# m4tx/idencomp

Measured on NVIDIA B200. Metric: fastq_compress_decompress_GBps, higher is better.
Workload: dtype u32

## Files before the change

idencomp_b200/csrc/idn_gpu.cu:

```cuda
#include "../../include/idn_gpu.h"

#include <algorithm>
#include <cstdarg>
#include <cstdio>
#include <chrono>
#include <cstring>
#include <string>
#include <vector>

#include "idn_fastq.cuh"
#include "idn_native.cuh"

using namespace idn;

namespace {

struct DevBuf {
    void* p = nullptr;
    size_t cap = 0;
    cudaError_t ensure(size_t n) {
        if (n <= cap) return cudaSuccess;
        if (p) cudaFree(p);
        p = nullptr;
        cap = 0;
// ... 36 lines not shown
        cudaFree(d_hvals);
        cudaFree(d_enc);
        cudaFree(d_dec);
        cudaFree(d_adirect);
        cudaFree(d_aenc);
        cudaFree(d_qwin);
        d_qwin = d_aenc = nullptr;
        d_map = d_hkeys = d_hvals = d_enc = d_dec = d_adirect = nullptr;
        used = false;
    }
};

constexpr uint32_t kMaxSlots = 1024;
constexpr uint64_t kDenseSpecLimit = 1ull << 22;
constexpr uint64_t kDirectSpecLimit = 1ull << 19;

}

struct idn_gpu_pipe;

struct idn_gpu_ctx {
    int device = 0;
    idn_gpu_pipe* pipe = nullptr;
    uint32_t pipe_blocks = 32;
    bool pipe_blocks_set = false;
    uint32_t* pipe_err_out = nullptr;
    cudaStream_t stream = nullptr;
    cudaEvent_t ev = nullptr;
    std::string err;
    uint64_t launches = 0;
    bool profiling = false;
    std::vector<cudaEvent_t> prof_pool;
    size_t prof_used = 0;
    struct ProfMark {
        const char* name;
        cudaEvent_t ev;
    };
    std::vector<ProfMark> prof_marks;
    struct HostPhase {
        const char* name;
        uint64_t n;
        double ms;
    };
    std::vector<HostPhase> host_phases;
    std::vector<ModelSlot> slots;
    ModelDev* d_models = nullptr;
    ModelDev d_models_host0{};
    int sm_count = 148;
    int32_t walk_mode = 0;
    uint32_t* d_crc_tab = nullptr;
    uint32_t* d_xpow = nullptr;
    uint32_t* d_crc_back = nullptr;
    bool enc_crc = true;
    DevBuf w_scratch, w_paylen, w_sizes, w_chosen, w_tiles, w_sliceoff, w_readblock, w_small, w_crcpart, w_crclen;
    DevBuf w_walkdone, w_blockadj;
    DevBuf w_lanefirst, w_laneoff, w_laneblock, w_blkinfo, w_nhdr, w_lanesym;
    uint32_t lane_syms = 2048;
    DevBuf f_text, f_tilecnt, f_tilebase, f_linestart, f_linefn, f_linestate, f_tilefn, f_tilestate, f_recscan, f_title, f_namelo,
        f_namelen, f_readlen, f_readoff, f_nameoff, f_names, f_acids, f_quals, f_err, f_fmtoff, f_fmttext;
    idn_fastq_info f_info{};
    uint64_t f_consumed = 0;
    DevBuf f_blockfirst, f_nxt;
    uint32_t f_blocks = 0;
    uint64_t f_reads_used = 0;
    DevBuf w_index;
    DevBuf w_blk;
    DevBuf s_acids, s_quals, s_readoff, s_blockfirst, s_prefix, s_names, s_nameoff, s_out, s_blockoff, s_crc, s_stats,
        s_sizes, s_blocks, s_blocklen, s_aout, s_qout, s_offout, s_status, s_idx;
    DevBuf w_bucket, w_list;
    bool bucket_pairs = true;
    uint64_t resident_bytes = 0;
    uint32_t resident_blocks = 0;
};

namespace {

int32_t fail(idn_gpu_ctx* c, int32_t code, const char* fmt, ...) {
    if (c) {
        char buf[512];
        va_list ap;
        va_start(ap, fmt);
        vsnprintf(buf, sizeof buf, fmt, ap);
        va_end(ap);
        c->err = buf;
    }
    return code;
}

#define CU(call)                                                                                       \
    do {                                                                                               \
        cudaError_t e__ = (call);                                                                      \
        if (e__ != cudaSuccess) {                                                                      \
            (void)cudaGetLastError();                                                                  \
            return fail(ctx, IDN_E_CUDA, "%s failed: %s (%s:%d)", #call, cudaGetErrorString(e__), __FILE__, \
                        __LINE__);                                                                     \
        }                                                                                              \
    } while (0)

#define LAUNCHED(name)                                                                             \
    do {                                                                                           \
        ctx->launches++;                                                                           \
        if (ctx->profiling) prof_mark(ctx, name, st);                                              \
        cudaError_t e__ = cudaGetLastError();                                                      \
        if (e__ != cudaSuccess)                                                                    \
            return fail(ctx, IDN_E_CUDA, "kernel launch failed: %s (%s:%d)", cudaGetErrorString(e__), \
                        __FILE__, __LINE__);                                                       \
// ... 88 lines not shown

using SP0 = StaticSpecs<1, 8, 0, 0, 1, 0, 0, 2, 6, 0>;
using SP1 = StaticSpecs<1, 8, 0, 0, 1, 0, 2, 1, 6, 0>;
using SP2 = StaticSpecs<0, 8, 0, 0, 0, 1, 0, 4, 0, 16>;
using SP3 = StaticSpecs<1, 4, 3, 2, 8, 1, 0, 4, 3, 16>;
using SP4 = StaticSpecs<0, 4, 1, 2, 0, 1, 0, 4, 3, 16>;
using SP5 = StaticSpecs<0, 8, 0, 0, 0, 1, 2, 4, 2, 8>;
using SP6 = StaticSpecs<0, 8, 0, 0, 0, 1, 0, 3, 0, 32>;
using SP7 = StaticSpecs<0, 8, 0, 0, 0, 1, 0, 4, 3, 16>;
constexpr int kNumStaticPairs = 8;
static const int32_t kStaticPairs[kNumStaticPairs][10] = {
    {1, 8, 0, 0, 1, 0, 0, 2, 6, 0}, {1, 8, 0, 0, 1, 0, 2, 1, 6, 0}, {0, 8, 0, 0, 0, 1, 0, 4, 0, 16}, {1, 4, 3, 2, 8, 1, 0, 4, 3, 16},
    {0, 4, 1, 2, 0, 1, 0, 4, 3, 16}, {0, 8, 0, 0, 0, 1, 2, 4, 2, 8}, {0, 8, 0, 0, 0, 1, 0, 3, 0, 32}, {0, 8, 0, 0, 0, 1, 0, 4, 3, 16}};

static int static_pair_index(const idn_gpu_ctx* ctx, int32_t acid_slot, int32_t q_slot) {
    if (!ctx->slots[acid_slot].dev.map || !ctx->slots[q_slot].dev.map || !ctx->slots[acid_slot].dev.adirect || !ctx->slots[q_slot].dev.qwin) return -1;
#ifndef IDN_NO_AENC
    if (!ctx->slots[acid_slot].dev.aenc) return -1;
#endif
    for (int i = 0; i < kNumStaticPairs; i++) {
        bool same = true;
        for (int k = 0; k < 5; k++)
            same = same && ctx->slots[acid_slot].spec_tuple[k] == kStaticPairs[i][k] && ctx->slots[q_slot].spec_tuple[k] == kStaticPairs[i][5 + k];
        if (same) return i;
    }
    return -1;
}

extern "C" int32_t idn_gpu_kernel_variant(const idn_gpu_ctx* ctx, idn_model_t acid_model, idn_model_t q_model) {
    if (!ctx) return -1;
    for (idn_model_t h : {acid_model, q_model})
        if (h < 0 || (size_t)h >= ctx->slots.size() || !ctx->slots[h].used) return -1;
    if (ctx->slots[acid_model].dev.type != IDN_MODEL_ACID || ctx->slots[q_model].dev.type != IDN_MODEL_QSCORE) return -1;
    return static_pair_index(ctx, acid_model, q_model);
}
extern "C" int32_t idn_gpu_kernel_variant_count(void) { return kNumStaticPairs; }

static unsigned debug_smem() {
    static const unsigned v = [] { const char* e = getenv("IDN_DEBUG_SMEM"); return e ? (unsigned)atoi(e) : 0u; }();
    return v;
}
#define IDN_LAUNCH_UNIFORM(idx, KERNEL, grid, st, ...)                                         \
    switch (idx) {                                                                             \
        case 0: KERNEL<true, SP0><<<grid, 128, debug_smem(), st>>>(__VA_ARGS__); break;                   \
        case 1: KERNEL<true, SP1><<<grid, 128, debug_smem(), st>>>(__VA_ARGS__); break;                   \
        case 2: KERNEL<true, SP2><<<grid, 128, debug_smem(), st>>>(__VA_ARGS__); break;                   \
        case 3: KERNEL<true, SP3><<<grid, 128, debug_smem(), st>>>(__VA_ARGS__); break;                   \
        case 4: KERNEL<true, SP4><<<grid, 128, debug_smem(), st>>>(__VA_ARGS__); break;                   \
        case 5: KERNEL<true, SP5><<<grid, 128, debug_smem(), st>>>(__VA_ARGS__); break;                   \
        case 6: KERNEL<true, SP6><<<grid, 128, debug_smem(), st>>>(__VA_ARGS__); break;                   \
        case 7: KERNEL<true, SP7><<<grid, 128, debug_smem(), st>>>(__VA_ARGS__); break;                   \
        default: KERNEL<true, DynSpecs><<<grid, 128, debug_smem(), st>>>(__VA_ARGS__); break;             \
    }

#define IDN_LAUNCH_LIST(idx, KERNEL, grid, st, ...)                                            \
    switch (idx) {                                                                             \
        case 0: KERNEL<SP0><<<grid, 128, debug_smem(), st>>>(__VA_ARGS__); break;                         \
        case 1: KERNEL<SP1><<<grid, 128, debug_smem(), st>>>(__VA_ARGS__); break;                         \
        case 2: KERNEL<SP2><<<grid, 128, debug_smem(), st>>>(__VA_ARGS__); break;                         \
        case 3: KERNEL<SP3><<<grid, 128, debug_smem(), st>>>(__VA_ARGS__); break;                         \
        case 4: KERNEL<SP4><<<grid, 128, debug_smem(), st>>>(__VA_ARGS__); break;                         \
        case 5: KERNEL<SP5><<<grid, 128, debug_smem(), st>>>(__VA_ARGS__); break;                         \
        case 6: KERNEL<SP6><<<grid, 128, debug_smem(), st>>>(__VA_ARGS__); break;                         \
        case 7: KERNEL<SP7><<<grid, 128, debug_smem(), st>>>(__VA_ARGS__); break;                         \
        default: KERNEL<DynSpecs><<<grid, 128, debug_smem(), st>>>(__VA_ARGS__); break;                   \
    }

extern "C" int32_t idn_gpu_abi_version(void) { return IDN_GPU_ABI_VERSION; }

extern "C" int32_t idn_gpu_device_count(void) {
    int n = 0;
    if (cudaGetDeviceCount(&n) != cudaSuccess) {
        (void)cudaGetLastError();
        return 0;
    }
    return n;
}

static void make_crc_tables(uint32_t* tab, uint32_t* xpow) {
    for (uint32_t i = 0; i < 256; i++) {
        uint32_t c = i;
        for (int k = 0; k < 8; k++) c = (c >> 1) ^ ((c & 1) ? 0xEDB88320u : 0);
        tab[i] = c;
    }
    auto mul = [](uint32_t a, uint32_t b) {
        uint32_t p = 0;
        for (int i = 0; i < 32; i++) {
            if (b & 0x80000000u) p ^= a;
            a = (a >> 1) ^ ((a & 1) ? 0xEDB88320u : 0);
            b <<= 1;
        }
        return p;
    };
    xpow[0] = 0x00800000u;
    for (int k = 1; k < 64; k++) xpow[k] = mul(xpow[k - 1], xpow[k - 1]);
}

static void make_crc_back_tables(const uint32_t* tab, const uint32_t* xpow, uint32_t* back ) {
    uint32_t rtop[256];
    for (uint32_t i = 0; i < 256; i++) rtop[tab[i] >> 24] = i;
    uint32_t* tinv = back;
    uint32_t* u = back + 256;
    for (uint32_t t = 0; t < 256; t++) tinv[t] = (tab[rtop[t]] << 8) | rtop[t];
    auto linv = [&](uint32_t v) { return (v << 8) ^ tinv[v >> 24]; };
    for (uint32_t b = 0; b < 256; b++) u[b] = linv(tab[b]);
    auto mul = [](uint32_t a, uint32_t b) {
// ... 1 lines not shown
        for (int i = 0; i < 32; i++) {
            if (b & 0x80000000u) p ^= a;
            a = (a >> 1) ^ ((a & 1) ? 0xEDB88320u : 0);
            b <<= 1;
        }
        return p;
    };
    uint32_t* xlen = back + 512;
    uint32_t x = 0x80000000u;
    for (uint32_t n = 0; n < kCrcLenTab; n++) {
        xlen[2 * n] = x;
        xlen[2 * n + 1] = mul(x, x);
        x = mul(x, xpow[0]);
    }
}

extern "C" int32_t idn_gpu_create(int32_t device, idn_gpu_ctx** out) {
    if (!out) return IDN_E_INVALID_ARG;
    *out = nullptr;
    int n = idn_gpu_device_count();
    if (n <= 0 || device < 0 || device >= n) return IDN_E_CUDA;
    idn_gpu_ctx* ctx = new idn_gpu_ctx();
    ctx->device = device;
    if (const char* pb = getenv("IDN_PIPE_BLOCKS")) {
        ctx->pipe_blocks = std::max(1, atoi(pb));
        ctx->pipe_blocks_set = true;
    }
    if (getenv("IDN_NO_BUCKETS")) ctx->bucket_pairs = false;
    if (const char* w = getenv("IDN_WALK")) ctx->walk_mode = strcmp(w, "serial") == 0 ? 1 : (strcmp(w, "fast") == 0 ? 2 : 0);
    auto bail = [&](const char* what) {
        fprintf(stderr, "idn_gpu_create: %s failed: %s\n", what, cudaGetErrorString(cudaGetLastError()));
        delete ctx;
        return (int32_t)IDN_E_CUDA;
    };
    if (cudaSetDevice(device) != cudaSuccess) return bail("cudaSetDevice");
    if (cudaDeviceGetAttribute(&ctx->sm_count, cudaDevAttrMultiProcessorCount, device) != cudaSuccess) return bail("cudaDeviceGetAttribute");
    if (cudaStreamCreateWithFlags(&ctx->stream, cudaStreamNonBlocking) != cudaSuccess) return bail("cudaStreamCreate");
    if (cudaEventCreateWithFlags(&ctx->ev, cudaEventDisableTiming | cudaEventBlockingSync) != cudaSuccess) return bail("cudaEventCreate");
    if (cudaMalloc(&ctx->d_models, sizeof(ModelDev) * kMaxSlots) != cudaSuccess) return bail("cudaMalloc");
    if (cudaMemset(ctx->d_models, 0, sizeof(ModelDev) * kMaxSlots) != cudaSuccess) return bail("cudaMemset");
    uint32_t tab[256], xpow[64];
    make_crc_tables(tab, xpow);
    if (cudaMalloc(&ctx->d_crc_tab, sizeof tab) != cudaSuccess) return bail("cudaMalloc");
    if (cudaMalloc(&ctx->d_xpow, sizeof xpow) != cudaSuccess) return bail("cudaMalloc");
    if (cudaMemcpy(ctx->d_crc_tab, tab, sizeof tab, cudaMemcpyHostToDevice) != cudaSuccess) return bail("cudaMemcpy");
    if (cudaMemcpy(ctx->d_xpow, xpow, sizeof xpow, cudaMemcpyHostToDevice) != cudaSuccess) return bail("cudaMemcpy");
    {
        std::vector<uint32_t> back(512 + 2 * kCrcLenTab);
        make_crc_back_tables(tab, xpow, back.data());
        if (cudaMalloc(&ctx->d_crc_back, back.size() * 4) != cudaSuccess) return bail("cudaMalloc");
        if (cudaMemcpy(ctx->d_crc_back, back.data(), back.size() * 4, cudaMemcpyHostToDevice) != cudaSuccess) return bail("cudaMemcpy");
    }
    if (getenv("IDN_NO_ENC_CRC")) ctx->enc_crc = false;
    *out = ctx;
    return IDN_OK;
}

static void pipe_destroy(idn_gpu_pipe* p);

extern "C" void idn_gpu_destroy(idn_gpu_ctx* ctx) {
    if (!ctx) return;
    cudaSetDevice(ctx->device);
    cudaDeviceSynchronize();
    for (auto& s : ctx->slots)
        if (s.used) s.free_all();
    DevBuf* bufs[] = {&ctx->w_scratch, &ctx->w_paylen,  &ctx->w_sizes,   &ctx->w_chosen,     &ctx->w_tiles,  &ctx->w_sliceoff,
                      &ctx->w_readblock, &ctx->w_small, &ctx->w_crcpart, &ctx->w_crclen,     &ctx->w_index,  &ctx->w_blk,
                      &ctx->w_lanefirst, &ctx->w_laneoff, &ctx->w_laneblock, &ctx->w_blkinfo, &ctx->w_nhdr, &ctx->w_lanesym, &ctx->w_walkdone, &ctx->w_blockadj,
                      &ctx->f_text, &ctx->f_tilecnt, &ctx->f_tilebase, &ctx->f_linestart, &ctx->f_linefn, &ctx->f_linestate, &ctx->f_tilefn,
                      &ctx->f_tilestate, &ctx->f_recscan, &ctx->f_title, &ctx->f_namelo, &ctx->f_namelen, &ctx->f_readlen, &ctx->f_readoff,
                      &ctx->f_nameoff, &ctx->f_names, &ctx->f_acids, &ctx->f_quals, &ctx->f_err, &ctx->f_fmtoff, &ctx->f_fmttext,
                      &ctx->f_blockfirst, &ctx->f_nxt, &ctx->w_bucket, &ctx->w_list,
                      &ctx->s_acids,   &ctx->s_quals,   &ctx->s_readoff, &ctx->s_blockfirst, &ctx->s_prefix, &ctx->s_names,
                      &ctx->s_nameoff, &ctx->s_out,     &ctx->s_blockoff, &ctx->s_crc,       &ctx->s_stats,  &ctx->s_sizes,
                      &ctx->s_blocks,  &ctx->s_blocklen, &ctx->s_aout,    &ctx->s_qout,    &ctx->s_offout,     &ctx->s_status, &ctx->s_idx};
    for (DevBuf* b : bufs) b->release();
    pipe_destroy(ctx->pipe);
    cudaFree(ctx->d_models);
    cudaFree(ctx->d_crc_tab);
    cudaFree(ctx->d_xpow);
    cudaFree(ctx->d_crc_back);
    if (ctx->ev) cudaEventDestroy(ctx->ev);
    if (ctx->stream) cudaStreamDestroy(ctx->stream);
    delete ctx;
}

extern "C" int32_t idn_gpu_host_alloc(uint64_t bytes, void** p) {
    if (!p) return IDN_E_INVALID_ARG;
    *p = nullptr;
    if (cudaHostAlloc(p, bytes ? bytes : 1, cudaHostAllocPortable) != cudaSuccess) {
        (void)cudaGetLastError();
        *p = nullptr;
        return IDN_E_CUDA;
    }
    return IDN_OK;
}
extern "C" void idn_gpu_host_free(void* p) {
    if (p) cudaFreeHost(p);
}

extern "C" int32_t idn_gpu_set_walk(idn_gpu_ctx* ctx, int32_t mode) {
    if (!ctx) return IDN_E_INVALID_ARG;
    if (mode < 0 || mode > 2) return fail(ctx, IDN_E_INVALID_ARG, "walk mode %d", mode);
    ctx->walk_mode = mode;
    return IDN_OK;
}
// ... 328 lines not shown
                                   uint32_t* block_crc, idn_compress_stats* stats_dev, cudaStream_t st);


extern "C" int32_t idn_gpu_compress_blocks_dev(idn_gpu_ctx* ctx, const idn_batch* batch, int32_t mode,
                                               const idn_model_t* models, uint32_t n_models, int32_t fast,
                                               const uint32_t* prefix_len, uint8_t* out, uint64_t out_cap,
                                               uint64_t* block_off, uint32_t* block_crc, idn_compress_stats* stats_dev,
                                               void* stream) {
    if (!ctx) return IDN_E_INVALID_ARG;
    int32_t rc = check_batch(ctx, batch);
    if (rc) return rc;
    rc = check_models(ctx, models, n_models);
    if (rc) return rc;
    if (mode != IDN_MODE_COMPAT && mode != IDN_MODE_NATIVE) return fail(ctx, IDN_E_UNSUPPORTED, "unknown mode %d", mode);
    if (!batch->block_first_read || !block_off || (!out && out_cap)) return fail(ctx, IDN_E_INVALID_ARG, "NULL argument");
    if (batch->n_blocks == 0) return fail(ctx, IDN_E_INVALID_ARG, "batch has no blocks");
    CU(cudaSetDevice(ctx->device));
    cudaStream_t st = as_stream(stream);
    PROF_BEGIN();
    const uint64_t R = batch->n_reads, S = batch->n_symbols;
    const uint32_t B = batch->n_blocks;
    const bool fuse_crc = ctx->enc_crc && batch->names == nullptr && R > 0;

    SmallParams sp;
    memset(&sp, 0, sizeof sp);
    uint32_t n_score = 0;
    for (uint32_t i = 0; i < n_models; i++) {
        uint32_t t = ctx->slots[models[i]].dev.type;
        if (sp.n_cand[t] >= (uint32_t)kMaxCand) return fail(ctx, IDN_E_UNSUPPORTED, "more than %d models of one type", kMaxCand);
        uint32_t k = sp.n_cand[t]++;
        sp.cand_model[t * kMaxCand + k] = models[i];
        sp.cand_index[t * kMaxCand + k] = (uint8_t)i;
    }
    if (R > 0 && (sp.n_cand[0] == 0 || sp.n_cand[1] == 0))
        return fail(ctx, IDN_E_INVALID_STATE, "need at least one acid model and one quality score model");
    if (fast && n_models != 2) return fail(ctx, IDN_E_INVALID_STATE, "fast mode needs exactly 2 models (compressor_block.rs:96)");
    for (uint32_t t = 0; t < 2; t++) {
        sp.has_sizes[t] = !fast && sp.n_cand[t] > 1;
        if (sp.has_sizes[t])
            for (uint32_t k = 0; k < sp.n_cand[t]; k++) {
                sp.cand_cols[t * kMaxCand + k] = n_score;
                sp.score_ids[n_score++] = sp.cand_model[t * kMaxCand + k];
            }
    }
    if (mode == IDN_MODE_NATIVE) return compress_native_dev(ctx, batch, sp, fast, prefix_len, out, out_cap, block_off, block_crc, stats_dev, st);
    rc = upload_small(ctx, sp, st);
    if (rc) return rc;
    SmallParams* dsp = ctx->w_small.as<SmallParams>();

    CU(ctx->w_scratch.ensure(4 * S + kSlotExtra * R + 16));
    CU(ctx->w_paylen.ensure((R + 1) * 4));
    CU(ctx->w_sliceoff.ensure((R + 2) * 8));
    CU(ctx->w_readblock.ensure((R + 1) * 4));
    const uint32_t n_tiles = (uint32_t)((R + kScanTile - 1) / kScanTile);
    CU(ctx->w_tiles.ensure(((size_t)n_tiles + 2) * 8));
    uint8_t* chosen = nullptr;
    uint8_t* switched = nullptr;
    if (!fast) {
        CU(ctx->w_chosen.ensure(4 * R + 16));
        chosen = ctx->w_chosen.as<uint8_t>();
        switched = chosen + 2 * R;
    }

    if (R > 0) {
        if (n_score) {
            CU(ctx->w_sizes.ensure(R * n_score * 4));
            rc = launch_score(ctx, sp.score_ids, n_score, batch, n_score, ctx->w_sizes.as<uint32_t>(), &dsp->err, st);
            if (rc) return rc;
        }
        if (!fast && n_score == 0) {
            CU(cudaMemsetAsync(chosen, 0, 4 * R, st));
            switch_single_kernel<<<(B + 127) / 128, 128, 0, st>>>(batch->block_first_read, B, switched, R);
            LAUNCHED("switch_single");
        } else if (!fast) {
            switch_kernel<<<2 * B, 32, 0, st>>>(ctx->w_sizes.as<uint32_t>(), n_score, dsp->cand_cols, dsp->n_cand,
                                                dsp->has_sizes, batch->block_first_read, B, chosen, switched, R);
            LAUNCHED("switch");
        }
        EncodeArgs ea;
        ea.models = ctx->d_models;
        ea.acids = batch->acids;
        ea.quals = batch->quals;
        ea.n_symbols = S;
        ea.read_off = batch->read_off;
        ea.n_reads = R;
        ea.fixed_acid = sp.cand_model[0];
        ea.fixed_q = sp.cand_model[kMaxCand];
        ea.chosen = chosen;
        ea.cand_model = dsp->cand_model;
        ea.scratch = ctx->w_scratch.as<uint8_t>();
        ea.pay_len = ctx->w_paylen.as<uint32_t>();
        ea.err = &dsp->err;
        ea.switched = switched;
        ea.cand_index = dsp->cand_index;
        ea.crc_back = nullptr;
        ea.xpow = ctx->d_xpow;
        ea.part_crc = nullptr;
        ea.part_len = nullptr;
        if (fuse_crc) {
            CU(ctx->w_crcpart.ensure((R + 1) * 4));
            CU(ctx->w_crclen.ensure((R + 1) * 8));
            ea.crc_back = ctx->d_crc_back;
            ea.part_crc = ctx->w_crcpart.as<uint32_t>();
            ea.part_len = ctx->w_crclen.as<unsigned long long>();
        }
        const bool uniform = !chosen || (sp.n_cand[0] == 1 && sp.n_cand[1] == 1);
        const ModelDev& hma = ctx->slots[sp.cand_model[0]].dev;
        const ModelDev& hmq = ctx->slots[sp.cand_model[kMaxCand]].dev;
        const unsigned egrid = (unsigned)((R + 127) / 128);
        const uint32_t n_pairs = sp.n_cand[0] * sp.n_cand[1];
        if (uniform) {
            IDN_LAUNCH_UNIFORM(static_pair_index(ctx, sp.cand_model[0], sp.cand_model[kMaxCand]), encode_kernel, egrid, st, ea, hma, hmq)
            LAUNCHED("encode");
        } else if (ctx->bucket_pairs && n_pairs <= kMaxPairs && R < 0xffffffffull) {
            CU(ctx->w_bucket.ensure(3 * kMaxPairs * 4));
            CU(ctx->w_list.ensure(R * 4 + 16));
            uint32_t* cnt = ctx->w_bucket.as<uint32_t>();
            uint32_t *base = cnt + kMaxPairs, *cursor = cnt + 2 * kMaxPairs;
            CU(cudaMemsetAsync(cnt, 0, kMaxPairs * 4, st));
            const EncodePairKey key{chosen, R, sp.n_cand[1]};
            const unsigned bgrid = (unsigned)((R + 255) / 256);
            bucket_count_kernel<<<bgrid, 256, 0, st>>>(key, R, n_pairs, cnt);
            LAUNCHED("bucket_count");
            bucket_base_kernel<<<1, 32, 0, st>>>(cnt, n_pairs, base, cursor);
            LAUNCHED("bucket_base");
            bucket_scatter_kernel<<<bgrid, 256, 0, st>>>(key, R, n_pairs, cursor, ctx->w_list.as<uint32_t>());
            LAUNCHED("bucket_scatter");
            ReadList rl{ctx->w_list.as<uint32_t>(), nullptr, nullptr};
            const unsigned lgrid = (unsigned)std::min<uint64_t>(egrid, (uint64_t)ctx->sm_count * IDN_ENC_MINB);
            for (uint32_t a = 0; a < sp.n_cand[0]; a++)
                for (uint32_t q = 0; q < sp.n_cand[1]; q++) {
                    const int32_t ia = sp.cand_model[a], iq = sp.cand_model[kMaxCand + q];
                    rl.base = base + a * sp.n_cand[1] + q;
                    rl.count = cnt + a * sp.n_cand[1] + q;
                    IDN_LAUNCH_LIST(static_pair_index(ctx, ia, iq), encode_list_kernel, lgrid, st, ea, ctx->slots[ia].dev, ctx->slots[iq].dev, rl)
                    LAUNCHED("encode");
                }
        } else {
            encode_kernel<false, DynSpecs><<<egrid, 128, 0, st>>>(ea, hma, hmq);
            LAUNCHED("encode");
        }
    }

    SliceSize fn{ctx->w_paylen.as<uint32_t>(), switched, R};
    unsigned long long* tiles = ctx->w_tiles.as<unsigned long long>();
    unsigned long long* slice_off = ctx->w_sliceoff.as<unsigned long long>();
    if (n_tiles) {
        scan_reduce_kernel<<<n_tiles, kScanBlock, 0, st>>>(fn, R, tiles);
        LAUNCHED("scan_reduce");
    }
    scan_tiles_kernel<<<1, kScanBlock, 0, st>>>(tiles, n_tiles);
    LAUNCHED("scan_tiles");
    if (n_tiles) {
        scan_apply_kernel<<<n_tiles, kScanBlock, 0, st>>>(fn, R, tiles, slice_off);
        LAUNCHED("scan_apply");
    } else {
        CU(cudaMemsetAsync(slice_off, 0, 8, st));
    }
    CU(ctx->w_blockadj.ensure(((size_t)B + 1) * 8));
    block_layout_kernel<<<1, 32, 0, st>>>(slice_off, batch->block_first_read, B, prefix_len, fast,
                                          reinterpret_cast<unsigned long long*>(block_off), out, out_cap, dsp->stats,
                                          ctx->w_blockadj.as<unsigned long long>());
    LAUNCHED("block_layout");
    if (R > 0) {
        read_block_kernel<<<B, 256, 0, st>>>(batch->block_first_read, B, ctx->w_readblock.as<uint32_t>());
        LAUNCHED("read_block");
        AssembleArgs aa;
        aa.read_off = batch->read_off;
        aa.n_reads = R;
        aa.pay_len = ctx->w_paylen.as<uint32_t>();
        aa.scratch = ctx->w_scratch.as<uint8_t>();
        aa.slice_off = slice_off;
        aa.block_adj = ctx->w_blockadj.as<unsigned long long>();
        aa.read_block = ctx->w_readblock.as<uint32_t>();
        aa.chosen = chosen;
        aa.switched = switched;
        aa.cand_index = dsp->cand_index;
        aa.out = out;
        aa.out_cap = out_cap;
        assemble_kernel<<<(unsigned)((R + 127) / 128), 128, 0, st>>>(aa);
        LAUNCHED("assemble");
        stats_kernel<<<592, 256, 0, st>>>(ctx->w_paylen.as<uint32_t>(), switched, R, dsp->stats);
        LAUNCHED("stats");
    }
    rc = idn_gpu_block_crc_dev_impl(ctx, batch, block_crc, out, reinterpret_cast<unsigned long long*>(block_off), out_cap, st, fuse_crc);
    if (rc) return rc;
    if (stats_dev) {
        finish_stats_kernel<<<1, 32, 0, st>>>(dsp->stats, &dsp->err, reinterpret_cast<unsigned long long*>(stats_dev), ctx->pipe_err_out);
        LAUNCHED("finish_stats");
    }
    return IDN_OK;
}

static int32_t launch_crc_read(idn_gpu_ctx* ctx, const uint8_t* acids, const uint8_t* quals, const unsigned long long* read_off,
                               const uint8_t* names, const unsigned long long* name_off, uint64_t n_reads,
                               const unsigned long long* n_reads_dev, const int32_t* status, uint64_t grid_reads, uint64_t avg_len,
                               cudaStream_t st, const uint32_t* run_flag = nullptr) {
    if (avg_len >= 1024) {
        crc_read_warp_kernel<<<(unsigned)((grid_reads * 32 + 127) / 128), 128, 0, st>>>(
            acids, quals, read_off, names, name_off, n_reads, n_reads_dev, status, ctx->d_crc_tab, ctx->d_xpow,
            ctx->w_crcpart.as<uint32_t>(), ctx->w_crclen.as<unsigned long long>(), run_flag);
    } else {
        const uint64_t tiles = (grid_reads + kCrcThreads - 1) / kCrcThreads;
        const unsigned cgrid = (unsigned)std::min<uint64_t>(tiles ? tiles : 1, (uint64_t)ctx->sm_count * 2);
        crc_read_kernel<<<cgrid, kCrcThreads, 0, st>>>(acids, quals, read_off, names, name_off, n_reads, n_reads_dev,
                                                                             status, ctx->d_crc_tab, ctx->d_xpow,
                                                                             ctx->w_crcpart.as<uint32_t>(),
                                                                             ctx->w_crclen.as<unsigned long long>(), run_flag);
    }
    LAUNCHED("crc_read");
    return IDN_OK;
}

static int32_t idn_gpu_block_crc_dev_impl(idn_gpu_ctx* ctx, const idn_batch* batch, uint32_t* block_crc, uint8_t* out,
                                          const unsigned long long* block_off, uint64_t out_cap, cudaStream_t st, bool have_partials) {
    const uint64_t R = batch->n_reads;
    CU(ctx->w_crcpart.ensure((R + 1) * 4));
    CU(ctx->w_crclen.ensure((R + 1) * 8));
    if (R > 0 && !have_partials) {
        int32_t rc = launch_crc_read(ctx, batch->acids, batch->quals, reinterpret_cast<const unsigned long long*>(batch->read_off),
                                     batch->names, reinterpret_cast<const unsigned long long*>(batch->name_off), R, nullptr, nullptr, R,
                                     batch->n_symbols / R, st);
        if (rc) return rc;
    }
    crc_block_kernel<<<batch->n_blocks, 256, 0, st>>>(ctx->w_crcpart.as<uint32_t>(), ctx->w_crclen.as<unsigned long long>(),
                                                      batch->block_first_read, batch->n_blocks, ctx->d_xpow, block_crc, out,
                                                      block_off, out_cap);
    LAUNCHED("crc_block");
    return IDN_OK;
}

template <class Fn>
static int32_t scan_u64(idn_gpu_ctx* ctx, Fn fn, uint64_t n, unsigned long long* out, cudaStream_t st) {
    const uint32_t n_tiles = (uint32_t)((n + kScanTile - 1) / kScanTile);
// ... 1201 lines not shown
```

idencomp_b200/csrc/idn_kernels.cuh:

```cuda
#pragma once
#include "idn_device.cuh"

namespace idn {

struct BackReader {
    const uint32_t* wp;
    uint32_t word;
    int lane;
    __device__ __forceinline__ void start(const uint8_t* last) {
        const uintptr_t a = reinterpret_cast<uintptr_t>(last);
        wp = reinterpret_cast<const uint32_t*>(a & ~(uintptr_t)3);
        lane = (int)(a & 3) + 4;
        word = 0;
    }
    __device__ __forceinline__ uint32_t get() {
        if (lane >= 4) {
            word = __ldg(wp);
            lane -= 4;
        }
        const uint32_t b = (word >> (8 * lane)) & 0xffu;
        if (--lane < 0) {
            lane = 7;
            wp--;
        }
// ... 452 lines not shown
#endif
#ifndef IDN_DEC_MINB
#define IDN_DEC_MINB 8
#endif
template <bool kUniform, class P>
__device__ __forceinline__ void encode_one(const EncodeArgs& A, const ModelDev& MA, const ModelDev& MQ, uint64_t r, const uint32_t* s_back) {
    int32_t ia = A.fixed_acid, iq = A.fixed_q;
    if (!kUniform && A.chosen) {
        ia = A.cand_model[A.chosen[r]];
        iq = A.cand_model[kMaxCand + A.chosen[A.n_reads + r]];
    }
    const ModelDev& ma = kUniform ? MA : A.models[ia];
    const ModelDev& mq = kUniform ? MQ : A.models[iq];
    const long long off = (long long)A.read_off[r];
    const uint32_t len = (uint32_t)(A.read_off[r + 1] - A.read_off[r]);
    EncStream S;
    S.begin(A.scratch + 4ull * A.read_off[r + 1] + kSlotExtra * (r + 1));
    EncCrc C{A.crc_back ? s_back : nullptr, s_back + 256, 0u, 0u};
    encode_read_body<P>(ma, mq, A.acids, A.quals, A.n_symbols, off, len, 0, len, S, C);
    if (A.crc_back) {
        uint32_t x1, x2;
        if (len < kCrcLenTab) {
            const uint2 x = __ldg(reinterpret_cast<const uint2*>(A.crc_back + 512) + len);
            x1 = x.x;
            x2 = x.y;
        } else {
            x1 = x8n_mod_p(len, A.xpow);
            x2 = gf2_mul(x1, x1);
        }
        A.part_crc[r] = len ? ~(gf2_mul(x1, C.bq) ^ gf2_mul(x2, ~C.ba)) : 0u;
        A.part_len[r] = 2ull * len;
    }
    S.flush_states();
    const uint32_t plen = S.total(A.scratch + 4ull * A.read_off[r + 1] + kSlotExtra * (r + 1));
    A.pay_len[r] = plen;
    S.out.push_u32_le(__byte_perm(len, 0, 0x0123));
    S.out.push_u32_le(__byte_perm(plen, 0, 0x0123));
    S.out.push_bits(2u, 8);
    S.out.drain();
    if (A.switched) {
        if (A.switched[A.n_reads + r]) {
            S.out.push_bits(((uint32_t)A.cand_index[kMaxCand + A.chosen[A.n_reads + r]] << 8) | 1u, 16);
            S.out.drain();
        }
        if (A.switched[r]) {
            S.out.push_bits(((uint32_t)A.cand_index[A.chosen[r]] << 8) | 1u, 16);
            S.out.drain();
        }
    }
    S.out.finish();
    if (S.bad) atomicOr(A.err, 1u);
}

template <bool kUniform, class P>
__global__ void __launch_bounds__(128, kUniform ? IDN_ENC_MINB : 1)
encode_kernel(EncodeArgs A, const ModelDev MA, const ModelDev MQ) {
    __shared__ uint32_t s_back[512];
    if (A.crc_back) {
        for (int i = threadIdx.x; i < 512; i += blockDim.x) s_back[i] = A.crc_back[i];
        __syncthreads();
    }
    uint64_t r = (uint64_t)blockIdx.x * blockDim.x + threadIdx.x;
    if (r >= A.n_reads) return;
    encode_one<kUniform, P>(A, MA, MQ, r, s_back);
}

template <class P>
__global__ void __launch_bounds__(128, IDN_ENC_MINB)
encode_list_kernel(EncodeArgs A, const ModelDev MA, const ModelDev MQ, ReadList L) {
    __shared__ uint32_t s_back[512];
    if (A.crc_back) {
        for (int i = threadIdx.x; i < 512; i += blockDim.x) s_back[i] = A.crc_back[i];
        __syncthreads();
    }
    const uint32_t n = *L.count;
    const uint32_t* __restrict__ list = L.list + *L.base;
    for (uint64_t i = (uint64_t)blockIdx.x * blockDim.x + threadIdx.x; i < n; i += (uint64_t)gridDim.x * blockDim.x)
        encode_one<true, P>(A, MA, MQ, list[i], s_back);
}

constexpr uint32_t kMaxPairs = 1024;

struct EncodePairKey {
    const uint8_t* chosen;
    uint64_t n_reads;
    uint32_t n_q;
    __device__ __forceinline__ uint32_t operator()(uint64_t r) const {
        return r < n_reads ? (uint32_t)chosen[r] * n_q + chosen[n_reads + r] : 0xffffffffu;
    }
};

template <class KeyFn>
__global__ void __launch_bounds__(256)
bucket_count_kernel(KeyFn key, uint64_t n, uint32_t n_pairs, uint32_t* __restrict__ cnt) {
    __shared__ uint32_t hist[kMaxPairs];
    for (uint32_t k = threadIdx.x; k < n_pairs; k += blockDim.x) hist[k] = 0;
    __syncthreads();
    const uint64_t r = (uint64_t)blockIdx.x * blockDim.x + threadIdx.x;
    const uint32_t k = r < n ? key(r) : 0xffffffffu;
    if (k < n_pairs) atomicAdd(&hist[k], 1u);
    __syncthreads();
    for (uint32_t j = threadIdx.x; j < n_pairs; j += blockDim.x)
        if (hist[j]) atomicAdd(&cnt[j], hist[j]);
}

__global__ void bucket_base_kernel(const uint32_t* __restrict__ cnt, uint32_t n_pairs, uint32_t* __restrict__ base, uint32_t* __restrict__ cursor) {
    if (threadIdx.x != 0 || blockIdx.x != 0) return;
    uint32_t acc = 0;
    for (uint32_t k = 0; k < n_pairs; k++) {
        base[k] = cursor[k] = acc;
// ... 111 lines not shown
    }
};

__global__ void __launch_bounds__(32)
block_layout_kernel(const unsigned long long* __restrict__ slice_off, const uint32_t* __restrict__ block_first,
                    uint32_t n_blocks, const uint32_t* __restrict__ prefix_len, int fast,
                    unsigned long long* __restrict__ block_off , uint8_t* __restrict__ out,
                    uint64_t out_cap, unsigned long long* __restrict__ stats ,
                    unsigned long long* __restrict__ block_adj ) {
    if (threadIdx.x != 0) return;
    unsigned long long pos = 0;
    for (uint32_t b = 0; b < n_blocks; b++) {
        block_off[b] = pos;
        unsigned long long body = slice_off[block_first[b + 1]] - slice_off[block_first[b]];
        bool empty = block_first[b + 1] == block_first[b];
        block_adj[b] = pos + 8 + (prefix_len ? prefix_len[b] : 0) + (fast ? 4 : 0) - slice_off[block_first[b]];
        unsigned long long extra = (prefix_len ? prefix_len[b] : 0) + ((fast && !empty) ? 4 : 0);
        unsigned long long length = body + extra;
        if (pos + 8 <= out_cap) {
            uint32_t l = (uint32_t)length;
            out[pos + 0] = (uint8_t)(l >> 24);
            out[pos + 1] = (uint8_t)(l >> 16);
            out[pos + 2] = (uint8_t)(l >> 8);
            out[pos + 3] = (uint8_t)l;
            uint64_t f = pos + 8 + (prefix_len ? prefix_len[b] : 0);
            if (fast && !empty && f + 4 <= out_cap) {
                out[f + 0] = 1;
                out[f + 1] = 0;
                out[f + 2] = 1;
                out[f + 3] = 1;
            }
        }
        pos += 8 + length;
    }
    block_off[n_blocks] = pos;
    stats[0] = pos;
}

struct AssembleArgs {
    const uint64_t* read_off;
    uint64_t n_reads;
    const uint32_t* pay_len;
    const uint8_t* scratch;
    const unsigned long long* slice_off;
    const unsigned long long* block_adj;
    const uint32_t* read_block;
    const uint8_t* chosen;
    const uint8_t* switched;
    const uint8_t* cand_index;
    uint8_t* out;
    uint64_t out_cap;
};

__device__ __forceinline__ void copy_bytes_words(uint8_t* __restrict__ d, const uint8_t* __restrict__ src, uint32_t n) {
    uint32_t head = (uint32_t)((4 - (reinterpret_cast<uintptr_t>(d) & 3)) & 3);
    if (head > n) head = n;
    for (uint32_t i = 0; i < head; i++) d[i] = src[i];
    const uint32_t words = (n - head) >> 2;
    const uint8_t* s2 = src + head;
    const uint32_t sh = (uint32_t)(reinterpret_cast<uintptr_t>(s2) & 3);
    const uint32_t* sw = reinterpret_cast<const uint32_t*>(s2 - sh);
    uint32_t* dw = reinterpret_cast<uint32_t*>(d + head);
    if (sh == 0) {
#pragma unroll 4
        for (uint32_t i = 0; i < words; i++) dw[i] = __ldg(sw + i);
    } else if (words) {
        uint32_t lo = __ldg(sw);
#pragma unroll 4
        for (uint32_t i = 0; i < words; i++) {
            uint32_t hi = __ldg(sw + i + 1);
            dw[i] = __funnelshift_r(lo, hi, 8 * sh);
            lo = hi;
        }
    }
    for (uint32_t i = head + 4 * words; i < n; i++) d[i] = src[i];
}

__global__ void __launch_bounds__(128)
assemble_kernel(AssembleArgs A) {
    uint64_t r = (uint64_t)blockIdx.x * blockDim.x + threadIdx.x;
    if (r >= A.n_reads) return;
    const unsigned long long dst = A.slice_off[r] + A.block_adj[A.read_block[r]];
    uint32_t nsw = 0;
    if (A.switched) nsw = A.switched[r] + A.switched[A.n_reads + r];
    const uint32_t total = 2u * nsw + 9u + A.pay_len[r];
    if (dst + total > A.out_cap) return;
    const uint8_t* src = A.scratch + 4ull * A.read_off[r + 1] + kSlotExtra * (r + 1) - total;
    copy_bytes_words(A.out + dst, src, total);
}

__global__ void read_block_kernel(const uint32_t* __restrict__ block_first, uint32_t n_blocks,
                                  uint32_t* __restrict__ read_block) {
    uint32_t b = blockIdx.x;
    if (b >= n_blocks) return;
    for (uint64_t r = block_first[b] + threadIdx.x; r < block_first[b + 1]; r += blockDim.x) read_block[r] = b;
}

__global__ void __launch_bounds__(256)
stats_kernel(const uint32_t* __restrict__ pay_len, const uint8_t* __restrict__ switched, uint64_t n_reads,
             unsigned long long* __restrict__ stats) {
    unsigned long long pay = 0, sa = 0, sq = 0;
    for (uint64_t r = (uint64_t)blockIdx.x * blockDim.x + threadIdx.x; r < n_reads; r += (uint64_t)gridDim.x * blockDim.x) {
        pay += pay_len[r];
        if (switched) {
            sa += switched[r];
            sq += switched[n_reads + r];
        }
    }
    for (int d = 16; d > 0; d >>= 1) {
        pay += __shfl_down_sync(0xffffffffu, pay, d);
        sa += __shfl_down_sync(0xffffffffu, sa, d);
        sq += __shfl_down_sync(0xffffffffu, sq, d);
    }
    if ((threadIdx.x & 31) == 0) {
        atomicAdd(&stats[1], sa);
        atomicAdd(&stats[2], sq);
        atomicAdd(&stats[3], pay);
    }
}

__global__ void finish_stats_kernel(const unsigned long long* __restrict__ stats, const uint32_t* __restrict__ err,
                                    unsigned long long* __restrict__ out, uint32_t* __restrict__ err_out) {
    if (threadIdx.x != 0 || blockIdx.x != 0) return;
    out[0] = stats[0];
    out[1] = stats[1];
    out[2] = stats[2];
    out[3] = stats[3];
    out[4] = stats[0];
    if (err_out) {
        err_out[0] = *err;
        err_out[1] = 0;
    }
}

__device__ __forceinline__ uint32_t gf2_mul(uint32_t a, uint32_t b) {
    uint32_t p = 0;
#pragma unroll 4
    for (int i = 0; i < 32; i++) {
        p ^= (0u - (b >> 31)) & a;
        a = (a >> 1) ^ ((0u - (a & 1u)) & 0xEDB88320u);
        b <<= 1;
// ... 1142 lines not shown
```

Measured before the change: 268.9.

## Fuse slice-offset scan and payload assembly into the uniform encode kernel

For uniform-model batches, the encode kernel now takes dynamic tile tickets and publishes per-tile payload sums. It runs a decoupled look-back scan in which each tile places the tile one resident wave behind it, copying that tile's payloads straight to the output. This replaces the separate scan_reduce/scan_tiles/scan_apply, block_layout and assemble launches with a block-adjust prescan and a small block_finish kernel. The goal is to cut kernel launches and a second pass over scratch. In exchange it adds spin-waits, release/acquire traffic and extra register/shared pressure inside the encode kernel, and the lag is derived from occupancy queries.

```diff
diff --git a/idencomp_b200/csrc/idn_gpu.cu b/idencomp_b200/csrc/idn_gpu.cu
--- a/idencomp_b200/csrc/idn_gpu.cu
+++ b/idencomp_b200/csrc/idn_gpu.cu
@@ -112,6 +112,9 @@
     uint32_t* d_xpow = nullptr;
     uint32_t* d_crc_back = nullptr;
     bool enc_crc = true;
+    bool fused_asm = true;
+    int32_t fused_lag = -1;
+    int32_t enc_resident[9] = {};
     DevBuf w_scratch, w_paylen, w_sizes, w_chosen, w_tiles, w_sliceoff, w_readblock, w_small, w_crcpart, w_crclen;
     DevBuf w_walkdone, w_blockadj;
     DevBuf w_lanefirst, w_laneoff, w_laneblock, w_blkinfo, w_nhdr, w_lanesym;
@@ -306,6 +309,32 @@
         case 7: KERNEL<true, SP7><<<grid, 128, debug_smem(), st>>>(__VA_ARGS__); break;                   \
         default: KERNEL<true, DynSpecs><<<grid, 128, debug_smem(), st>>>(__VA_ARGS__); break;             \
     }
+
+template <class P>
+static cudaError_t encode_resident(int* n) {
+    return cudaOccupancyMaxActiveBlocksPerMultiprocessor(n, encode_kernel<true, P>, 128, debug_smem());
+}
+static cudaError_t fused_lag(idn_gpu_ctx* ctx, int idx, uint32_t* lag) {
+    if (ctx->fused_lag >= 0) {
+        *lag = (uint32_t)ctx->fused_lag;
+        return cudaSuccess;
+    }
+    int& n = ctx->enc_resident[idx < 0 || idx >= kNumStaticPairs ? kNumStaticPairs : idx];
+    cudaError_t e = cudaSuccess;
+    if (n == 0) switch (idx) {
+            case 0: e = encode_resident<SP0>(&n); break;
+            case 1: e = encode_resident<SP1>(&n); break;
+            case 2: e = encode_resident<SP2>(&n); break;
+            case 3: e = encode_resident<SP3>(&n); break;
+            case 4: e = encode_resident<SP4>(&n); break;
+            case 5: e = encode_resident<SP5>(&n); break;
+            case 6: e = encode_resident<SP6>(&n); break;
+            case 7: e = encode_resident<SP7>(&n); break;
+            default: e = encode_resident<DynSpecs>(&n); break;
+        }
+    *lag = (uint32_t)(n * ctx->sm_count);
+    return e;
+}
 
 #define IDN_LAUNCH_LIST(idx, KERNEL, grid, st, ...)                                            \
     switch (idx) {                                                                             \
@@ -413,6 +442,8 @@
         if (cudaMemcpy(ctx->d_crc_back, back.data(), back.size() * 4, cudaMemcpyHostToDevice) != cudaSuccess) return bail("cudaMemcpy");
     }
     if (getenv("IDN_NO_ENC_CRC")) ctx->enc_crc = false;
+    if (getenv("IDN_NO_FUSED_ASSEMBLY")) ctx->fused_asm = false;
+    if (const char* l = getenv("IDN_FUSED_LAG")) ctx->fused_lag = std::max(0, atoi(l));
     *out = ctx;
     return IDN_OK;
 }
@@ -847,14 +878,40 @@
     CU(ctx->w_paylen.ensure((R + 1) * 4));
     CU(ctx->w_sliceoff.ensure((R + 2) * 8));
     CU(ctx->w_readblock.ensure((R + 1) * 4));
-    const uint32_t n_tiles = (uint32_t)((R + kScanTile - 1) / kScanTile);
-    CU(ctx->w_tiles.ensure(((size_t)n_tiles + 2) * 8));
     uint8_t* chosen = nullptr;
     uint8_t* switched = nullptr;
     if (!fast) {
         CU(ctx->w_chosen.ensure(4 * R + 16));
         chosen = ctx->w_chosen.as<uint8_t>();
         switched = chosen + 2 * R;
+    }
+    unsigned long long* slice_off = ctx->w_sliceoff.as<unsigned long long>();
+    const bool uniform = !chosen || (sp.n_cand[0] == 1 && sp.n_cand[1] == 1);
+    FusedAsm fa{};
+    const unsigned egrid = (unsigned)((R + 127) / 128);
+    bool fused = R > 0 && uniform && ctx->fused_asm;
+    if (fused) {
+        CU(fused_lag(ctx, static_pair_index(ctx, sp.cand_model[0], sp.cand_model[kMaxCand]), &fa.lag));
+        fused = ctx->fused_lag >= 0 || egrid >= 4ull * fa.lag;
+    }
+    if (fused) {
+        CU(ctx->w_blockadj.ensure((2 * (size_t)B + 1) * 8));
+        unsigned long long* adj = ctx->w_blockadj.as<unsigned long long>();
+        block_adj_kernel<<<1, kScanBlock, 0, st>>>(batch->block_first_read, B, prefix_len, fast, adj, adj + B);
+        LAUNCHED("block_adj");
+        read_block_kernel<<<B, 256, 0, st>>>(batch->block_first_read, B, ctx->w_readblock.as<uint32_t>());
+        LAUNCHED("read_block");
+        CU(ctx->w_tiles.ensure(((size_t)egrid + 1) * 8));
+        CU(cudaMemsetAsync(ctx->w_tiles.p, 0, ((size_t)egrid + 1) * 8, st));
+        fa.status = ctx->w_tiles.as<unsigned long long>();
+        fa.ticket = reinterpret_cast<uint32_t*>(fa.status + egrid);
+        fa.n_tiles = egrid;
+        fa.block_adj = adj;
+        fa.read_block = ctx->w_readblock.as<uint32_t>();
+        fa.block_first = batch->block_first_read;
+        fa.slice_off = slice_off;
+        fa.out = out;
+        fa.out_cap = out_cap;
     }
 
     if (R > 0) {
@@ -899,13 +956,11 @@
             ea.part_crc = ctx->w_crcpart.as<uint32_t>();
             ea.part_len = ctx->w_crclen.as<unsigned long long>();
         }
-        const bool uniform = !chosen || (sp.n_cand[0] == 1 && sp.n_cand[1] == 1);
         const ModelDev& hma = ctx->slots[sp.cand_model[0]].dev;
         const ModelDev& hmq = ctx->slots[sp.cand_model[kMaxCand]].dev;
-        const unsigned egrid = (unsigned)((R + 127) / 128);
         const uint32_t n_pairs = sp.n_cand[0] * sp.n_cand[1];
         if (uniform) {
-            IDN_LAUNCH_UNIFORM(static_pair_index(ctx, sp.cand_model[0], sp.cand_model[kMaxCand]), encode_kernel, egrid, st, ea, hma, hmq)
+            IDN_LAUNCH_UNIFORM(static_pair_index(ctx, sp.cand_model[0], sp.cand_model[kMaxCand]), encode_kernel, egrid, st, ea, hma, hmq, fa)
             LAUNCHED("encode");
         } else if (ctx->bucket_pairs && n_pairs <= kMaxPairs && R < 0xffffffffull) {
             CU(ctx->w_bucket.ensure(3 * kMaxPairs * 4));
@@ -932,49 +987,59 @@
                     LAUNCHED("encode");
                 }
         } else {
-            encode_kernel<false, DynSpecs><<<egrid, 128, 0, st>>>(ea, hma, hmq);
+            encode_kernel<false, DynSpecs><<<egrid, 128, 0, st>>>(ea, hma, hmq, fa);
             LAUNCHED("encode");
         }
     }
 
-    SliceSize fn{ctx->w_paylen.as<uint32_t>(), switched, R};
-    unsigned long long* tiles = ctx->w_tiles.as<unsigned long long>();
-    unsigned long long* slice_off = ctx->w_sliceoff.as<unsigned long long>();
-    if (n_tiles) {
-        scan_reduce_kernel<<<n_tiles, kScanBlock, 0, st>>>(fn, R, tiles);
-        LAUNCHED("scan_reduce");
-    }
-    scan_tiles_kernel<<<1, kScanBlock, 0, st>>>(tiles, n_tiles);
-    LAUNCHED("scan_tiles");
-    if (n_tiles) {
-        scan_apply_kernel<<<n_tiles, kScanBlock, 0, st>>>(fn, R, tiles, slice_off);
-        LAUNCHED("scan_apply");
+    if (fused) {
+        block_finish_kernel<<<(B + 128) / 128, 128, 0, st>>>(slice_off, batch->block_first_read, B, prefix_len, fast,
+                                                            ctx->w_blockadj.as<unsigned long long>() + B,
+                                                            reinterpret_cast<unsigned long long*>(block_off), out, out_cap, dsp->stats);
+        LAUNCHED("block_finish");
     } else {
-        CU(cudaMemsetAsync(slice_off, 0, 8, st));
-    }
-    CU(ctx->w_blockadj.ensure(((size_t)B + 1) * 8));
-    block_layout_kernel<<<1, 32, 0, st>>>(slice_off, batch->block_first_read, B, prefix_len, fast,
-                                          reinterpret_cast<unsigned long long*>(block_off), out, out_cap, dsp->stats,
-                                          ctx->w_blockadj.as<unsigned long long>());
-    LAUNCHED("block_layout");
+        SliceSize fn{ctx->w_paylen.as<uint32_t>(), switched, R};
+        const uint32_t n_tiles = (uint32_t)((R + kScanTile - 1) / kScanTile);
+        CU(ctx->w_tiles.ensure(((size_t)n_tiles + 2) * 8));
+        unsigned long long* tiles = ctx->w_tiles.as<unsigned long long>();
+        if (n_tiles) {
+            scan_reduce_kernel<<<n_tiles, kScanBlock, 0, st>>>(fn, R, tiles);
+            LAUNCHED("scan_reduce");
+        }
+        scan_tiles_kernel<<<1, kScanBlock, 0, st>>>(tiles, n_tiles);
+        LAUNCHED("scan_tiles");
+        if (n_tiles) {
+            scan_apply_kernel<<<n_tiles, kScanBlock, 0, st>>>(fn, R, tiles, slice_off);
+            LAUNCHED("scan_apply");
+        } else {
+            CU(cudaMemsetAsync(slice_off, 0, 8, st));
+        }
+        CU(ctx->w_blockadj.ensure(((size_t)B + 1) * 8));
+        block_layout_kernel<<<1, 32, 0, st>>>(slice_off, batch->block_first_read, B, prefix_len, fast,
+                                              reinterpret_cast<unsigned long long*>(block_off), out, out_cap, dsp->stats,
+                                              ctx->w_blockadj.as<unsigned long long>());
+        LAUNCHED("block_layout");
+        if (R > 0) {
+            read_block_kernel<<<B, 256, 0, st>>>(batch->block_first_read, B, ctx->w_readblock.as<uint32_t>());
+            LAUNCHED("read_block");
+            AssembleArgs aa;
+            aa.read_off = batch->read_off;
+            aa.n_reads = R;
+            aa.pay_len = ctx->w_paylen.as<uint32_t>();
+            aa.scratch = ctx->w_scratch.as<uint8_t>();
+            aa.slice_off = slice_off;
+            aa.block_adj = ctx->w_blockadj.as<unsigned long long>();
+            aa.read_block = ctx->w_readblock.as<uint32_t>();
+            aa.chosen = chosen;
+            aa.switched = switched;
+            aa.cand_index = dsp->cand_index;
+            aa.out = out;
+            aa.out_cap = out_cap;
+            assemble_kernel<<<(unsigned)((R + 127) / 128), 128, 0, st>>>(aa);
+            LAUNCHED("assemble");
+        }
+    }
     if (R > 0) {
-        read_block_kernel<<<B, 256, 0, st>>>(batch->block_first_read, B, ctx->w_readblock.as<uint32_t>());
-        LAUNCHED("read_block");
-        AssembleArgs aa;
-        aa.read_off = batch->read_off;
-        aa.n_reads = R;
-        aa.pay_len = ctx->w_paylen.as<uint32_t>();
-        aa.scratch = ctx->w_scratch.as<uint8_t>();
-        aa.slice_off = slice_off;
-        aa.block_adj = ctx->w_blockadj.as<unsigned long long>();
-        aa.read_block = ctx->w_readblock.as<uint32_t>();
-        aa.chosen = chosen;
-        aa.switched = switched;
-        aa.cand_index = dsp->cand_index;
-        aa.out = out;
-        aa.out_cap = out_cap;
-        assemble_kernel<<<(unsigned)((R + 127) / 128), 128, 0, st>>>(aa);
-        LAUNCHED("assemble");
         stats_kernel<<<592, 256, 0, st>>>(ctx->w_paylen.as<uint32_t>(), switched, R, dsp->stats);
         LAUNCHED("stats");
     }
diff --git a/idencomp_b200/csrc/idn_kernels.cuh b/idencomp_b200/csrc/idn_kernels.cuh
--- a/idencomp_b200/csrc/idn_kernels.cuh
+++ b/idencomp_b200/csrc/idn_kernels.cuh
@@ -528,10 +528,36 @@
     if (S.bad) atomicOr(A.err, 1u);
 }
 
+struct FusedAsm {
+    unsigned long long* status;
+    uint32_t* ticket;
+    uint32_t n_tiles;
+    uint32_t lag;
+    const unsigned long long* block_adj;
+    const uint32_t* read_block;
+    const uint32_t* block_first;
+    unsigned long long* slice_off;
+    uint8_t* out;
+    uint64_t out_cap;
+};
+__device__ __forceinline__ void fused_assembly(const EncodeArgs& A, const FusedAsm& F, uint32_t t);
+
 template <bool kUniform, class P>
 __global__ void __launch_bounds__(128, kUniform ? IDN_ENC_MINB : 1)
-encode_kernel(EncodeArgs A, const ModelDev MA, const ModelDev MQ) {
+encode_kernel(const __grid_constant__ EncodeArgs A, const ModelDev MA, const ModelDev MQ, const __grid_constant__ FusedAsm F) {
     __shared__ uint32_t s_back[512];
+    __shared__ uint32_t s_tile;
+    if (kUniform && F.status) {
+        if (threadIdx.x == 0) s_tile = atomicAdd(F.ticket, 1u);
+        if (A.crc_back)
+            for (int i = threadIdx.x; i < 512; i += blockDim.x) s_back[i] = A.crc_back[i];
+        __syncthreads();
+        const uint64_t r = (uint64_t)s_tile * blockDim.x + threadIdx.x;
+        if (r < A.n_reads) encode_one<kUniform, P>(A, MA, MQ, r, s_back);
+        __syncthreads();
+        fused_assembly(A, F, s_tile);
+        return;
+    }
     if (A.crc_back) {
         for (int i = threadIdx.x; i < 512; i += blockDim.x) s_back[i] = A.crc_back[i];
         __syncthreads();
@@ -749,10 +775,17 @@
     uint64_t out_cap;
 };
 
-__device__ __forceinline__ void copy_bytes_words(uint8_t* __restrict__ d, const uint8_t* __restrict__ src, uint32_t n) {
+template <bool kNc, class T>
+__device__ __forceinline__ T ld_src(const T* p) {
+    if constexpr (kNc) return __ldg(p);
+    else return *p;
+}
+
+template <bool kNc = true>
+__device__ __forceinline__ void copy_bytes_words(uint8_t* __restrict__ d, const uint8_t* src, uint32_t n) {
     uint32_t head = (uint32_t)((4 - (reinterpret_cast<uintptr_t>(d) & 3)) & 3);
     if (head > n) head = n;
-    for (uint32_t i = 0; i < head; i++) d[i] = src[i];
+    for (uint32_t i = 0; i < head; i++) d[i] = ld_src<kNc>(src + i);
     const uint32_t words = (n - head) >> 2;
     const uint8_t* s2 = src + head;
     const uint32_t sh = (uint32_t)(reinterpret_cast<uintptr_t>(s2) & 3);
@@ -760,17 +793,17 @@
     uint32_t* dw = reinterpret_cast<uint32_t*>(d + head);
     if (sh == 0) {
 #pragma unroll 4
-        for (uint32_t i = 0; i < words; i++) dw[i] = __ldg(sw + i);
+        for (uint32_t i = 0; i < words; i++) dw[i] = ld_src<kNc>(sw + i);
     } else if (words) {
-        uint32_t lo = __ldg(sw);
+        uint32_t lo = ld_src<kNc>(sw);
 #pragma unroll 4
         for (uint32_t i = 0; i < words; i++) {
-            uint32_t hi = __ldg(sw + i + 1);
+            uint32_t hi = ld_src<kNc>(sw + i + 1);
             dw[i] = __funnelshift_r(lo, hi, 8 * sh);
             lo = hi;
         }
     }
-    for (uint32_t i = head + 4 * words; i < n; i++) d[i] = src[i];
+    for (uint32_t i = head + 4 * words; i < n; i++) d[i] = ld_src<kNc>(src + i);
 }
 
 __global__ void __launch_bounds__(128)
@@ -784,6 +817,141 @@
     if (dst + total > A.out_cap) return;
     const uint8_t* src = A.scratch + 4ull * A.read_off[r + 1] + kSlotExtra * (r + 1) - total;
     copy_bytes_words(A.out + dst, src, total);
+}
+
+__global__ void __launch_bounds__(kScanBlock)
+block_adj_kernel(const uint32_t* __restrict__ block_first, uint32_t n_blocks, const uint32_t* __restrict__ prefix_len, int fast,
+                 unsigned long long* __restrict__ block_adj , unsigned long long* __restrict__ hdr ) {
+    __shared__ unsigned long long smem[kScanBlock / 32];
+    __shared__ unsigned long long total;
+    unsigned long long carry = 0;
+    for (uint32_t base = 0; base < n_blocks; base += kScanBlock) {
+        const uint32_t b = base + threadIdx.x;
+        const unsigned long long pl = b < n_blocks && prefix_len ? prefix_len[b] : 0;
+        const bool empty = b < n_blocks && block_first[b + 1] == block_first[b];
+        const unsigned long long v = b < n_blocks ? 8 + pl + ((fast && !empty) ? 4 : 0) : 0;
+        const unsigned long long h = carry + block_exclusive_scan(v, &total, smem);
+        if (b < n_blocks) {
+            hdr[b] = h;
+            block_adj[b] = h + 8 + pl + (fast ? 4 : 0);
+        }
+        carry += total;
+        __syncthreads();
+    }
+    if (threadIdx.x == 0) hdr[n_blocks] = carry;
+}
+
+__global__ void __launch_bounds__(128)
+block_finish_kernel(const unsigned long long* __restrict__ slice_off, const uint32_t* __restrict__ block_first, uint32_t n_blocks,
+                    const uint32_t* __restrict__ prefix_len, int fast, const unsigned long long* __restrict__ hdr,
+                    unsigned long long* __restrict__ block_off, uint8_t* __restrict__ out, uint64_t out_cap,
+                    unsigned long long* __restrict__ stats) {
+    const uint32_t b = blockIdx.x * blockDim.x + threadIdx.x;
+    if (b > n_blocks) return;
+    const unsigned long long pos = slice_off[block_first[b]] + hdr[b];
+    block_off[b] = pos;
+    if (b == n_blocks) {
+        stats[0] = pos;
+        return;
+    }
+    const bool empty = block_first[b + 1] == block_first[b];
+    const unsigned long long pl = prefix_len ? prefix_len[b] : 0;
+    const unsigned long long length = slice_off[block_first[b + 1]] - slice_off[block_first[b]] + pl + ((fast && !empty) ? 4 : 0);
+    if (pos + 8 <= out_cap) {
+        const uint32_t l = (uint32_t)length;
+        out[pos + 0] = (uint8_t)(l >> 24);
+        out[pos + 1] = (uint8_t)(l >> 16);
+        out[pos + 2] = (uint8_t)(l >> 8);
+        out[pos + 3] = (uint8_t)l;
+        const uint64_t f = pos + 8 + pl;
+        if (fast && !empty && f + 4 <= out_cap) {
+            out[f + 0] = 1;
+            out[f + 1] = 0;
+            out[f + 2] = 1;
+            out[f + 3] = 1;
+        }
+    }
+}
+
+constexpr unsigned long long kTileAgg = 1ull << 62, kTileInc = 2ull << 62, kTileVal = kTileAgg - 1;
+
+__device__ __forceinline__ void st_release_gpu(unsigned long long* p, unsigned long long v) {
+    asm volatile("st.release.gpu.global.u64 [%0], %1;" ::"l"(p), "l"(v) : "memory");
+}
+__device__ __forceinline__ unsigned long long ld_acquire_gpu(const unsigned long long* p) {
+    unsigned long long v;
+    asm volatile("ld.acquire.gpu.global.u64 %0, [%1];" : "=l"(v) : "l"(p) : "memory");
+    return v;
+}
+__device__ __forceinline__ unsigned long long wait_status(const unsigned long long* p) {
+    unsigned long long s = ld_acquire_gpu(p);
+    for (uint32_t ns = 32; s == 0; ns = ns < 1024 ? 2 * ns : ns) {
+        __nanosleep(ns);
+        s = ld_acquire_gpu(p);
+    }
+    return s;
+}
+
+__device__ __forceinline__ unsigned long long warp_sum_u64(unsigned long long v) {
+    for (int d = 16; d > 0; d >>= 1) v += __shfl_xor_sync(0xffffffffu, v, d);
+    return v;
+}
+
+__device__ __forceinline__ void fused_place_tile(const EncodeArgs& A, const FusedAsm& F, uint32_t u) {
+    __shared__ unsigned long long s_warp[4];
+    __shared__ unsigned long long s_pre;
+    const uint32_t lane = threadIdx.x & 31, wid = threadIdx.x >> 5;
+    if (threadIdx.x == 0) wait_status(F.status + u);
+    __syncthreads();
+    const uint64_t r = (uint64_t)u * 128 + threadIdx.x;
+    const SliceSize fn{A.pay_len, A.switched, A.n_reads};
+    const unsigned long long v = r < A.n_reads ? fn(r) : 0;
+    unsigned long long inc = v;
+    for (int d = 1; d < 32; d <<= 1) {
+        const unsigned long long o = __shfl_up_sync(0xffffffffu, inc, d);
+        if (lane >= (uint32_t)d) inc += o;
+    }
+    if (lane == 31) s_warp[wid] = inc;
+    __syncthreads();
+    unsigned long long ex = inc - v;
+    for (uint32_t w = 0; w < wid; w++) ex += s_warp[w];
+    if (wid == 0) {
+        const unsigned long long total = s_warp[0] + s_warp[1] + s_warp[2] + s_warp[3];
+        unsigned long long pre = 0;
+        for (long long top = (long long)u - 1;; top -= 32) {
+            const long long i = top - (long long)lane;
+            const unsigned long long s = i >= 0 ? wait_status(F.status + i) : kTileInc;
+            const uint32_t inc_lanes = __ballot_sync(0xffffffffu, s >= kTileInc);
+            const uint32_t k = inc_lanes ? __ffs(inc_lanes) - 1 : 32;
+            pre += warp_sum_u64(lane <= k ? (s & kTileVal) : 0);
+            if (inc_lanes) break;
+        }
+        if (lane == 0) {
+            st_release_gpu(F.status + u, kTileInc | (pre + total));
+            s_pre = pre;
+            if (u == F.n_tiles - 1) F.slice_off[A.n_reads] = pre + total;
+        }
+    }
+    __syncthreads();
+    if (r >= A.n_reads) return;
+    const unsigned long long so = s_pre + ex;
+    const uint32_t b = __ldg(F.read_block + r);
+    if (__ldg(F.block_first + b) == r) F.slice_off[r] = so;
+    const unsigned long long dst = so + __ldg(F.block_adj + b);
+    if (dst + v > F.out_cap) return;
+    const uint8_t* src = A.scratch + 4ull * A.read_off[r + 1] + kSlotExtra * (r + 1) - v;
+    copy_bytes_words<false>(F.out + dst, src, (uint32_t)v);
+}
+
+__device__ __forceinline__ void fused_assembly(const EncodeArgs& A, const FusedAsm& F, uint32_t t) {
+    __shared__ unsigned long long s_red[4];
+    const uint64_t r = (uint64_t)t * 128 + threadIdx.x;
+    const unsigned long long v = warp_sum_u64(r < A.n_reads ? SliceSize{A.pay_len, A.switched, A.n_reads}(r) : 0);
+    if ((threadIdx.x & 31) == 0) s_red[threadIdx.x >> 5] = v;
+    __syncthreads();
+    if (threadIdx.x == 0) st_release_gpu(F.status + t, kTileAgg | (s_red[0] + s_red[1] + s_red[2] + s_red[3]));
+    if (t >= F.lag) fused_place_tile(A, F, t - F.lag);
+    if (t + F.lag >= F.n_tiles && F.lag > 0) fused_place_tile(A, F, t);
 }
 
 __global__ void read_block_kernel(const uint32_t* __restrict__ block_first, uint32_t n_blocks,
```

Result: faster. 275.6, median of 6 (+2.5%).
